# culiver/VAR

Hardware: AMD Instinct MI355X
Metric: 256x256 images/sec (CFG=1.5) VAR-d16 (higher is better)
Workload: dtype f32

## Files before the change

### var_amd/csrc/winograd.hip

```cpp
#include "common.h"

namespace {

constexpr int WG_PT = 18;
constexpr int WG_NDMA = 21;
constexpr int WG_STAGE = WG_NDMA * 16 * 64;
constexpr int WG_ZSTR = 20;
constexpr int WG_LDS = 2 * WG_STAGE;
static_assert(8 * 64 * WG_ZSTR * 4 <= WG_LDS, "epilogue exchange must fit in the K-loop stages");

struct WinoP {
    const float* in; const float* u; const float* bias; const float* resid; float* out; double* gn_part;
    int H, W, Cin, Cout, ncg, pw, ppi;
};

__device__ __forceinline__ void wg_wait_dma_barrier() { asm volatile("s_waitcnt vmcnt(0)\n\ts_barrier" ::: "memory"); }

__device__ __forceinline__ int wg_swz(int pix) { return (pix >> 1) & 3; }

__global__ void __launch_bounds__(256, 2) k_conv3x3_wino(WinoP p) {
    extern __shared__ __attribute__((aligned(16))) float smem[];
    const int tid = threadIdx.x, lane = tid & 63, wave = __builtin_amdgcn_readfirstlane(tid >> 6);
    const int r16 = lane & 15, kq = lane >> 4;
    int lin;
    {
        const int nwg = gridDim.x, bid = blockIdx.x, q = nwg >> 3, rem = nwg & 7, xcd = bid & 7, loc = bid >> 3;
        lin = (xcd < rem ? xcd * (q + 1) : rem * (q + 1) + (xcd - rem) * q) + loc;
    }
    const int cg = lin % p.ncg, pidx = lin / p.ncg, b = pidx / p.ppi, pi = pidx - b * p.ppi, py = pi / p.pw, px = pi - py * p.pw;
    const int y0 = py * 16, x0 = px * 16, c0 = cg * 32;
    const int H = p.H, W = p.W, Cin = p.Cin, Cout = p.Cout, nk = Cin >> 4;

    const int64_t img = (int64_t)H * W * Cin;
    const __amdgpu_buffer_rsrc_t rsrc = __builtin_amdgcn_make_buffer_rsrc((void*)(p.in + (int64_t)b * img), 0, (int)(img * 4), 0x00020000);
    uint32_t doff[6];
#pragma unroll
    for (int i = 0; i < 6; ++i) {
        const int pix = (wave + 4 * i) * 16 + (lane >> 2), c = lane & 3;
        const int yy = y0 - 1 + pix / WG_PT, xx = x0 - 1 + pix % WG_PT;
        const bool ok = pix < WG_PT * WG_PT && (unsigned)yy < (unsigned)H && (unsigned)xx < (unsigned)W;
        doff[i] = ok ? (uint32_t)((((int64_t)yy * W + xx) * Cin + ((c ^ wg_swz(pix)) << 2)) * 4) : 0x80000000u;
    }
    const uint32_t lds0 = (uint32_t)(uintptr_t)(__attribute__((address_space(3))) void*)smem;
    auto dma = [&](int kt, int st) {
#pragma unroll
        for (int i = 0; i < 6; ++i)
            if (wave + 4 * i < WG_NDMA) vh_dma16_buf(rsrc, doff[i], (uint32_t)kt * 64u, lds0 + st * WG_STAGE + (wave + 4 * i) * 1024);
    };

    const uint32_t ustr_xi = (uint32_t)nk * Cout * 64, ustr_kt = (uint32_t)Cout * 64;
    const __amdgpu_buffer_rsrc_t ursrc = __builtin_amdgcn_make_buffer_rsrc((void*)p.u, 0, (int)(16 * ustr_xi), 0x00020000);
    const uint32_t uoff = (uint32_t)((c0 + r16) * 16 + 4 * kq) * 4u;
    auto load_u = [&](int kt, f32x4 (&u)[4][2]) {
#pragma unroll
        for (int j = 0; j < 4; ++j)
#pragma unroll
            for (int cb = 0; cb < 2; ++cb)
                u[j][cb] = __builtin_bit_cast(f32x4, __builtin_amdgcn_raw_buffer_load_b128(
                    ursrc, uoff, __builtin_amdgcn_readfirstlane((uint32_t)(4 * wave + j) * ustr_xi + (uint32_t)kt * ustr_kt + cb * 1024u), 0));
    };

    const int ra = wave == 3 ? 1 : (wave == 2 ? 2 : wave), rb = wave == 0 ? 2 : (wave == 1 ? 2 : (wave == 2 ? 1 : 3));
    const float sg = wave == 1 ? 1.0f : -1.0f;
    uint32_t roff[2][4];
#pragma unroll
    for (int c = 0; c < 4; ++c) {
        const int pa = (2 * (r16 >> 3) + ra) * WG_PT + 2 * (r16 & 7) + c, pb = (2 * (r16 >> 3) + rb) * WG_PT + 2 * (r16 & 7) + c;
        roff[0][c] = (uint32_t)(pa * 64 + ((kq ^ wg_swz(pa)) << 4));
        roff[1][c] = (uint32_t)(pb * 64 + ((kq ^ wg_swz(pb)) << 4));
    }

    f32x4 acc[4][4][2];
#pragma unroll
    for (int j = 0; j < 4; ++j)
#pragma unroll
        for (int tb = 0; tb < 4; ++tb)
#pragma unroll
            for (int cb = 0; cb < 2; ++cb) acc[j][tb][cb] = f32x4{0.f, 0.f, 0.f, 0.f};

    auto compute = [&](int st, const f32x4 (&u)[4][2]) {
        const char* sb = (const char*)smem + st * WG_STAGE;
#pragma unroll
        for (int tb = 0; tb < 4; ++tb) {
            f32x4 da[4], db[4];
#pragma unroll
            for (int c = 0; c < 4; ++c) {
                da[c] = *(const f32x4*)(sb + roff[0][c] + tb * 72 * 64);
                db[c] = *(const f32x4*)(sb + roff[1][c] + tb * 72 * 64);
            }
#pragma unroll
            for (int s = 0; s < 4; ++s) {
                float e[4];
#pragma unroll
                for (int c = 0; c < 4; ++c) e[c] = __builtin_fmaf(sg, db[c][s], da[c][s]);
                const float v[4] = {e[0] - e[2], e[1] + e[2], e[2] - e[1], e[1] - e[3]};
#pragma unroll
                for (int j = 0; j < 4; ++j)
#pragma unroll
                    for (int cb = 0; cb < 2; ++cb) acc[j][tb][cb] = __builtin_amdgcn_mfma_f32_16x16x4f32(u[j][cb][s], v[j], acc[j][tb][cb], 0, 0, 0);
            }
            __builtin_amdgcn_sched_barrier(0);
        }
    };

    f32x4 u[4][2];
    dma(0, 0);
    wg_wait_dma_barrier();
    int kt = 0;
    for (; kt + 1 < nk; kt += 2) {
        load_u(kt, u); dma(kt + 1, 1);
        compute(0, u);
        wg_wait_dma_barrier();
        load_u(kt + 1, u); if (kt + 2 < nk) dma(kt + 2, 0);
        compute(1, u);
        wg_wait_dma_barrier();
    }
    if (kt < nk) { load_u(kt, u); compute(0, u); wg_wait_dma_barrier(); }

    float* zb = smem;
    const int et = tid & 63, eq = tid >> 6;
    const int ety = et >> 3, etx = et & 7;
    const int64_t obase = (((int64_t)b * H + y0 + 2 * ety) * W + x0 + 2 * etx) * Cout;
    const int nblk = p.gn_part ? (H * W) >> 7 : 0;
#pragma unroll
    for (int cb = 0; cb < 2; ++cb) {
#pragma unroll
        for (int tb = 0; tb < 4; ++tb) {
            const f32x4 m0 = acc[0][tb][cb], m1 = acc[1][tb][cb], m2 = acc[2][tb][cb], m3 = acc[3][tb][cb];
            const f32x4 z0 = (m0 + m1) + m2, z1 = (m1 - m2) - m3;
            const int t = tb * 16 + r16;
            *(f32x4*)(zb + ((wave * 2 + 0) * 64 + t) * WG_ZSTR + 4 * kq) = z0;
            *(f32x4*)(zb + ((wave * 2 + 1) * 64 + t) * WG_ZSTR + 4 * kq) = z1;
        }
        __syncthreads();
        f32x4 z[4][2];
#pragma unroll
        for (int i = 0; i < 4; ++i)
#pragma unroll
            for (int bb = 0; bb < 2; ++bb) z[i][bb] = *(const f32x4*)(zb + ((i * 2 + bb) * 64 + et) * WG_ZSTR + 4 * eq);
        const int co = c0 + cb * 16 + 4 * eq;
        const f32x4 b4 = *(const f32x4*)(p.bias + co);
        double gs[4] = {0.0, 0.0, 0.0, 0.0}, gq[4] = {0.0, 0.0, 0.0, 0.0};
#pragma unroll
        for (int a = 0; a < 2; ++a)
#pragma unroll
            for (int bb = 0; bb < 2; ++bb) {
                const f32x4 yv = a == 0 ? (z[0][bb] + z[1][bb]) + z[2][bb] : (z[1][bb] - z[2][bb]) - z[3][bb];
                f32x4 v = yv + b4;
                const int64_t o = obase + ((int64_t)a * W + bb) * Cout + co;
                if (p.resid) v = *(const f32x4*)(p.resid + o) + v;
                *(f32x4*)(p.out + o) = v;
#pragma unroll
                for (int e = 0; e < 4; ++e) { const double d = (double)v[e]; gs[e] += d; gq[e] += d * d; }
            }
        if (p.gn_part) {
#pragma unroll
            for (int off = 16; off >= 1; off >>= 1)
#pragma unroll
                for (int e = 0; e < 4; ++e) { gs[e] += __shfl_xor(gs[e], off, 64); gq[e] += __shfl_xor(gq[e], off, 64); }
            if ((lane & 31) == 0) {
                double* g = p.gn_part + (((int64_t)b * nblk + 2 * pi + (lane >> 5)) * Cout + co) * 2;
#pragma unroll
                for (int e = 0; e < 4; ++e) { g[2 * e] = gs[e]; g[2 * e + 1] = gq[e]; }
            }
        }
        if (cb == 0) __syncthreads();
    }
}

}

extern "C" int varhip_conv3x3_wino_nhwc_f32(const float* in, const float* u, const float* bias, const float* resid, float* out, double* gn_part,
                                            int B, int H, int W, int Cin, int Cout, varhip_stream_t stream) {
    if (!in || !u || !bias || !out || B <= 0 || H <= 0 || W <= 0 || Cin <= 0 || Cout <= 0) return VARHIP_EINVAL;
    if ((H & 15) || (W & 15) || (Cin & 31) || (Cout & 31)) return VARHIP_EINVAL;
    if ((((uintptr_t)in | (uintptr_t)u | (uintptr_t)bias | (uintptr_t)out | (uintptr_t)resid) & 15)) return VARHIP_EINVAL;
    if ((int64_t)H * W * Cin * 4 >= (1ll << 31) || 64ll * Cin * Cout >= (1ll << 31) || (int64_t)B * H * W >= (1ll << 31))
        return VARHIP_EINVAL;
    const int ppi = (H / 16) * (W / 16), ncg = Cout / 32;
    const int64_t nwg = (int64_t)B * ppi * ncg;
    if (nwg >= (1ll << 31)) return VARHIP_EINVAL;
    WinoP p{};
    p.in = in; p.u = u; p.bias = bias; p.resid = resid; p.out = out; p.gn_part = gn_part;
    p.H = H; p.W = W; p.Cin = Cin; p.Cout = Cout; p.ncg = ncg; p.pw = W / 16; p.ppi = ppi;
    const double npix = (double)B * H * W;
    VhScope scope(VH_FAM_CONV_WINO, (hipStream_t)stream, 2.0 * (npix / 4.0) * 16.0 * Cin * Cout,
                  4.0 * (npix * Cin + npix * Cout * (resid ? 2.0 : 1.0) + 16.0 * Cin * Cout));
    hipLaunchKernelGGL(k_conv3x3_wino, dim3((unsigned)nwg), dim3(256), WG_LDS, (hipStream_t)stream, p);
    return vh_launch_status();
}
```

Baseline: 153.2.

## Interleave U-weight loads and input DMA into the Winograd MFMA loop; template epilogue

Moves the per-k-tile weight (U) loads and the next-stage input DMA into the compute loop, so that each j-slice of U is refetched right after its last MFMA use. The barrier's wait is relaxed to vmcnt(8) so the in-flight U loads are not drained at each barrier. Bias and residual are prefetched during the final k-tile to hide epilogue latency. The kernel is templated on residual and GroupNorm use to drop runtime branches, and the GN partial reduction now uses a transpose-style shuffle tree so fewer doubles are shuffled. It also adds env-controlled debug variants that skip work, which raises register pressure and brings a risk of counter-ordering mistakes.

```diff
diff --git a/var_amd/csrc/winograd.hip b/var_amd/csrc/winograd.hip
--- a/var_amd/csrc/winograd.hip
+++ b/var_amd/csrc/winograd.hip
@@ -1,3 +1,6 @@
+#include <cstdlib>
+#include <type_traits>
+
 #include "common.h"
 
 namespace {
@@ -14,10 +17,13 @@
     int H, W, Cin, Cout, ncg, pw, ppi;
 };
 
-__device__ __forceinline__ void wg_wait_dma_barrier() { asm volatile("s_waitcnt vmcnt(0)\n\ts_barrier" ::: "memory"); }
+__device__ __forceinline__ void wg_wait_dma_barrier() { asm volatile("s_waitcnt vmcnt(8)\n\ts_barrier" ::: "memory"); }
+
+constexpr int WG_KO_NOEPI = 1, WG_KO_NOGN = 2, WG_KO_NORES = 4, WG_KO_NOBTDB = 8;
 
 __device__ __forceinline__ int wg_swz(int pix) { return (pix >> 1) & 3; }
 
+template <bool RES, bool GN, int KO>
 __global__ void __launch_bounds__(256, 2) k_conv3x3_wino(WinoP p) {
     extern __shared__ __attribute__((aligned(16))) float smem[];
     const int tid = threadIdx.x, lane = tid & 63, wave = __builtin_amdgcn_readfirstlane(tid >> 6);
@@ -51,14 +57,16 @@
     const uint32_t ustr_xi = (uint32_t)nk * Cout * 64, ustr_kt = (uint32_t)Cout * 64;
     const __amdgpu_buffer_rsrc_t ursrc = __builtin_amdgcn_make_buffer_rsrc((void*)p.u, 0, (int)(16 * ustr_xi), 0x00020000);
     const uint32_t uoff = (uint32_t)((c0 + r16) * 16 + 4 * kq) * 4u;
-    auto load_u = [&](int kt, f32x4 (&u)[4][2]) {
-#pragma unroll
-        for (int j = 0; j < 4; ++j)
-#pragma unroll
-            for (int cb = 0; cb < 2; ++cb)
-                u[j][cb] = __builtin_bit_cast(f32x4, __builtin_amdgcn_raw_buffer_load_b128(
-                    ursrc, uoff, __builtin_amdgcn_readfirstlane((uint32_t)(4 * wave + j) * ustr_xi + (uint32_t)kt * ustr_kt + cb * 1024u), 0));
-    };
+    f32x4 u[4][2];
+    auto load_u = [&](int kt, int j) {
+#pragma unroll
+        for (int cb = 0; cb < 2; ++cb)
+            u[j][cb] = __builtin_bit_cast(f32x4, __builtin_amdgcn_raw_buffer_load_b128(
+                ursrc, uoff, __builtin_amdgcn_readfirstlane((uint32_t)(4 * wave + j) * ustr_xi + (uint32_t)kt * ustr_kt + cb * 1024u), 0));
+    };
+    dma(0, 0);
+#pragma unroll
+    for (int j = 0; j < 4; ++j) { load_u(0, j); __builtin_amdgcn_sched_barrier(0); }
 
     const int ra = wave == 3 ? 1 : (wave == 2 ? 2 : wave), rb = wave == 0 ? 2 : (wave == 1 ? 2 : (wave == 2 ? 1 : 3));
     const float sg = wave == 1 ? 1.0f : -1.0f;
@@ -78,7 +86,20 @@
 #pragma unroll
             for (int cb = 0; cb < 2; ++cb) acc[j][tb][cb] = f32x4{0.f, 0.f, 0.f, 0.f};
 
-    auto compute = [&](int st, const f32x4 (&u)[4][2]) {
+    const int et = tid & 63, eq = tid >> 6;
+    const int ety = et >> 3, etx = et & 7;
+    const int64_t obase = (((int64_t)b * H + y0 + 2 * ety) * W + x0 + 2 * etx) * Cout + c0 + 4 * eq;
+    f32x4 b4[2], rs[2][2][2];
+    auto epi_load = [&](int j) {
+        if constexpr (KO & WG_KO_NOEPI) return;
+        if (j == 0) { b4[0] = *(const f32x4*)(p.bias + c0 + 4 * eq); b4[1] = *(const f32x4*)(p.bias + c0 + 16 + 4 * eq); }
+        if constexpr (RES) {
+#pragma unroll
+            for (int bb = 0; bb < 2; ++bb) rs[j >> 1][j & 1][bb] = *(const f32x4*)(p.resid + obase + ((int64_t)(j & 1) * W + bb) * Cout + (j >> 1) * 16);
+        }
+    };
+
+    auto compute = [&](int st, int kt_dma, int kt_u, auto last) {
         const char* sb = (const char*)smem + st * WG_STAGE;
 #pragma unroll
         for (int tb = 0; tb < 4; ++tb) {
@@ -88,40 +109,57 @@
                 da[c] = *(const f32x4*)(sb + roff[0][c] + tb * 72 * 64);
                 db[c] = *(const f32x4*)(sb + roff[1][c] + tb * 72 * 64);
             }
-#pragma unroll
-            for (int s = 0; s < 4; ++s) {
-                float e[4];
-#pragma unroll
-                for (int c = 0; c < 4; ++c) e[c] = __builtin_fmaf(sg, db[c][s], da[c][s]);
-                const float v[4] = {e[0] - e[2], e[1] + e[2], e[2] - e[1], e[1] - e[3]};
-#pragma unroll
-                for (int j = 0; j < 4; ++j)
-#pragma unroll
-                    for (int cb = 0; cb < 2; ++cb) acc[j][tb][cb] = __builtin_amdgcn_mfma_f32_16x16x4f32(u[j][cb][s], v[j], acc[j][tb][cb], 0, 0, 0);
+            float e[4][4];
+            if constexpr (!(KO & WG_KO_NOBTDB)) {
+#pragma unroll
+                for (int c = 0; c < 4; ++c)
+#pragma unroll
+                    for (int s = 0; s < 4; ++s) e[c][s] = __builtin_fmaf(sg, db[c][s], da[c][s]);
+            }
+#pragma unroll
+            for (int j = 0; j < 4; ++j) {
+#pragma unroll
+                for (int s = 0; s < 4; ++s) {
+                    float v;
+                    if constexpr (KO & WG_KO_NOBTDB) v = (j & 1) ? db[j][s] : da[j][s];
+                    else v = j == 0 ? e[0][s] - e[2][s] : (j == 1 ? e[1][s] + e[2][s] : (j == 2 ? e[2][s] - e[1][s] : e[1][s] - e[3][s]));
+#pragma unroll
+                    for (int cb = 0; cb < 2; ++cb) acc[j][tb][cb] = __builtin_amdgcn_mfma_f32_16x16x4f32(u[j][cb][s], v, acc[j][tb][cb], 0, 0, 0);
+                }
+                if (tb == 3) {
+                    __builtin_amdgcn_sched_barrier(0);
+                    if constexpr (decltype(last)::value) epi_load(j); else load_u(kt_u, j);
+                }
             }
             __builtin_amdgcn_sched_barrier(0);
-        }
-    };
-
-    f32x4 u[4][2];
-    dma(0, 0);
+            if (tb == 0 && !decltype(last)::value) dma(kt_dma, st ^ 1);
+        }
+    };
+
     wg_wait_dma_barrier();
     int kt = 0;
-    for (; kt + 1 < nk; kt += 2) {
-        load_u(kt, u); dma(kt + 1, 1);
-        compute(0, u);
+    for (; kt + 2 < nk; kt += 2) {
+        compute(0, kt + 1, kt + 1, std::false_type{});
         wg_wait_dma_barrier();
-        load_u(kt + 1, u); if (kt + 2 < nk) dma(kt + 2, 0);
-        compute(1, u);
+        compute(1, kt + 2, kt + 2, std::false_type{});
         wg_wait_dma_barrier();
     }
-    if (kt < nk) { load_u(kt, u); compute(0, u); wg_wait_dma_barrier(); }
+    compute(0, kt + 1, kt + 1, std::false_type{});
+    wg_wait_dma_barrier();
+    compute(1, 0, 0, std::true_type{});
+    __builtin_amdgcn_s_barrier();
+    if constexpr (KO & WG_KO_NOEPI) {
+#pragma unroll
+        for (int j = 0; j < 4; ++j)
+#pragma unroll
+            for (int tb = 0; tb < 4; ++tb)
+#pragma unroll
+                for (int cb = 0; cb < 2; ++cb) asm volatile("" :: "v"(acc[j][tb][cb]));
+        return;
+    }
 
     float* zb = smem;
-    const int et = tid & 63, eq = tid >> 6;
-    const int ety = et >> 3, etx = et & 7;
-    const int64_t obase = (((int64_t)b * H + y0 + 2 * ety) * W + x0 + 2 * etx) * Cout;
-    const int nblk = p.gn_part ? (H * W) >> 7 : 0;
+    const int nblk = (H * W) >> 7;
 #pragma unroll
     for (int cb = 0; cb < 2; ++cb) {
 #pragma unroll
@@ -139,30 +177,34 @@
 #pragma unroll
             for (int bb = 0; bb < 2; ++bb) z[i][bb] = *(const f32x4*)(zb + ((i * 2 + bb) * 64 + et) * WG_ZSTR + 4 * eq);
         const int co = c0 + cb * 16 + 4 * eq;
-        const f32x4 b4 = *(const f32x4*)(p.bias + co);
         double gs[4] = {0.0, 0.0, 0.0, 0.0}, gq[4] = {0.0, 0.0, 0.0, 0.0};
 #pragma unroll
         for (int a = 0; a < 2; ++a)
 #pragma unroll
             for (int bb = 0; bb < 2; ++bb) {
                 const f32x4 yv = a == 0 ? (z[0][bb] + z[1][bb]) + z[2][bb] : (z[1][bb] - z[2][bb]) - z[3][bb];
-                f32x4 v = yv + b4;
-                const int64_t o = obase + ((int64_t)a * W + bb) * Cout + co;
-                if (p.resid) v = *(const f32x4*)(p.resid + o) + v;
+                f32x4 v = yv + b4[cb];
+                const int64_t o = obase + ((int64_t)a * W + bb) * Cout + cb * 16;
+                if constexpr (RES) v = rs[cb][a][bb] + v;
                 *(f32x4*)(p.out + o) = v;
-#pragma unroll
-                for (int e = 0; e < 4; ++e) { const double d = (double)v[e]; gs[e] += d; gq[e] += d * d; }
-            }
-        if (p.gn_part) {
-#pragma unroll
-            for (int off = 16; off >= 1; off >>= 1)
-#pragma unroll
-                for (int e = 0; e < 4; ++e) { gs[e] += __shfl_xor(gs[e], off, 64); gq[e] += __shfl_xor(gq[e], off, 64); }
-            if ((lane & 31) == 0) {
-                double* g = p.gn_part + (((int64_t)b * nblk + 2 * pi + (lane >> 5)) * Cout + co) * 2;
-#pragma unroll
-                for (int e = 0; e < 4; ++e) { g[2 * e] = gs[e]; g[2 * e + 1] = gq[e]; }
-            }
+                if constexpr (GN) {
+#pragma unroll
+                    for (int e = 0; e < 4; ++e) { const double d = (double)v[e]; gs[e] += d; gq[e] += d * d; }
+                }
+            }
+        if constexpr (GN) {
+            const double t8[8] = {gs[0], gq[0], gs[1], gq[1], gs[2], gq[2], gs[3], gq[3]};
+            const bool h4 = lane & 16, h3 = lane & 8, h2 = lane & 4;
+            double r4[4], r2[2], r1;
+#pragma unroll
+            for (int i = 0; i < 4; ++i) r4[i] = (h4 ? t8[4 + i] : t8[i]) + __shfl_xor(h4 ? t8[i] : t8[4 + i], 16, 64);
+#pragma unroll
+            for (int i = 0; i < 2; ++i) r2[i] = (h3 ? r4[2 + i] : r4[i]) + __shfl_xor(h3 ? r4[i] : r4[2 + i], 8, 64);
+            r1 = (h2 ? r2[1] : r2[0]) + __shfl_xor(h2 ? r2[0] : r2[1], 4, 64);
+            r1 += __shfl_xor(r1, 2, 64);
+            r1 += __shfl_xor(r1, 1, 64);
+            if ((lane & 3) == 0)
+                p.gn_part[(((int64_t)b * nblk + 2 * pi + (lane >> 5)) * Cout + co) * 2 + ((lane >> 2) & 7)] = r1;
         }
         if (cb == 0) __syncthreads();
     }
@@ -186,6 +228,12 @@
     const double npix = (double)B * H * W;
     VhScope scope(VH_FAM_CONV_WINO, (hipStream_t)stream, 2.0 * (npix / 4.0) * 16.0 * Cin * Cout,
                   4.0 * (npix * Cin + npix * Cout * (resid ? 2.0 : 1.0) + 16.0 * Cin * Cout));
-    hipLaunchKernelGGL(k_conv3x3_wino, dim3((unsigned)nwg), dim3(256), WG_LDS, (hipStream_t)stream, p);
+    static const int dbg = [] { const char* e = getenv("VARHIP_WINO_DBG"); return e ? atoi(e) : 0; }();
+    const bool res = resid && !(dbg & WG_KO_NORES), gn = gn_part && !(dbg & WG_KO_NOGN);
+    if ((dbg & WG_KO_NOBTDB) && !(res && gn)) return VARHIP_EINVAL;
+    auto kfn = (dbg & WG_KO_NOEPI) ? k_conv3x3_wino<false, false, WG_KO_NOEPI> : (dbg & WG_KO_NOBTDB) ? k_conv3x3_wino<true, true, WG_KO_NOBTDB>
+             : res ? (gn ? k_conv3x3_wino<true, true, 0> : k_conv3x3_wino<true, false, 0>)
+                   : (gn ? k_conv3x3_wino<false, true, 0> : k_conv3x3_wino<false, false, 0>);
+    hipLaunchKernelGGL(kfn, dim3((unsigned)nwg), dim3(256), WG_LDS, (hipStream_t)stream, p);
     return vh_launch_status();
 }
```

Result: faster. 156.3, median of 6 (+2.0%).
